# galatolofederico/clip-glass

Hardware: AMD Instinct MI355X
Metric: candidate latents scored/sec (GAN→CLIP fitness), StyleGAN2_ffhq_d pop=64 (higher is better)
Workload: dtype f16; 1 GPU; StyleGAN2_ffhq_d: StyleGAN2 config-f 1024px G+D + CLIP ViT-B/32, pop=64 per GPU, batch_size=4, n_obj=2; pop_per_gpu=64, global_pop=64, batch_size=4, parallelism=population-shard x1, device=AMD Radeon Graphics (gfx950:sramecc+:xnack-), 256 CUs, hbm_gib=288

## Files before the change

clip_glass_amd/csrc/conv_down64.hip:

```cpp
#include "common.h"
#include "kernels.h"

namespace {
constexpr int TW = 29, CIN = 64, COUT = 128;
constexpr int ROWB = 64 * 128;
constexpr int V_BYTES = 4 * ROWB;
constexpr int A_BYTES = 8 * ROWB;
constexpr int XS_BYTES = 2 * 32 * 128;
constexpr int O_BYTES = 2 * 32 * 256;
constexpr int OFF_A = V_BYTES, OFF_XS = OFF_A + A_BYTES, OFF_O = OFF_XS + XS_BYTES, OFF_C = OFF_O + O_BYTES;
constexpr int LDS_BYTES = OFF_C + COUT * 4;

__device__ __forceinline__ int vaddr(int row, int col, int cg) { return row * ROWB + ((col ^ ((col >> 2) & 1)) << 7) + (cg << 4); }
__device__ __forceinline__ int aaddr(int rslot, int slot, int lc) { return rslot * ROWB + (slot << 7) + ((lc ^ ((slot >> 1) & 7)) << 4); }
__device__ __forceinline__ int oaddr(int row, int px, int c16) { return row * (32 * 256) + (px << 8) + ((c16 ^ (px & 15)) << 4); }
__device__ __forceinline__ h8 fir4(h8 a, h8 b, h8 c, h8 d) {
    const half_t q = (half_t)0.125f, t = (half_t)0.375f;
    const h8 k125 = {q, q, q, q, q, q, q, q}, k375 = {t, t, t, t, t, t, t, t};
    return __builtin_elementwise_fma(b + c, k375, (a + d) * k125);
}
__device__ __forceinline__ int opaque(int v) { asm volatile("" : "+v"(v)); return v; }
__device__ __forceinline__ int uni(int v) { return __builtin_amdgcn_readfirstlane(v); }
struct RSet { h8 a[4]; h8 x; int b, tx, s, valid; };
}

struct Down64Params {
    const half_t* h;
    const half_t* xs;
    const half_t* w1;
    const half_t* ws;
    const float* b1;
    half_t* y;
    int B, R;
};

__global__ __launch_bounds__(512, 1) void conv_down64_kernel(Down64Params p, int tiles_x, int SY, int n_steps, int per_block) {
    extern __shared__ __attribute__((aligned(16))) char smem[];
    char* Vs = smem;
    char* As = smem + OFF_A;
    char* Xs = smem + OFF_XS;
    char* Os = smem + OFF_O;
    float* Cb = (float*)(smem + OFF_C);
    const int R = p.R, Ro = R >> 1;
    const int first = blockIdx.x * per_block;
    const int last = min(first + per_block, n_steps);
    if (first >= last) return;
    const h8 zero = {0, 0, 0, 0, 0, 0, 0, 0};

    int nx_left = last - first, nx_prime = 1, nx_b, nx_tx, nx_s;
    {
        const int per_img = tiles_x * SY;
        nx_b = uni(first / per_img);
        const int rem = first - nx_b * per_img;
        nx_tx = uni(rem / SY);
        nx_s = uni(rem - nx_tx * SY);
    }
    const int total = nx_left + 1 + (nx_s + nx_left - 1) / SY;

    auto issue = [&](RSet& Rg) {
        Rg.b = nx_b; Rg.tx = nx_tx;
        if (nx_prime) {
            Rg.s = nx_s - 1; Rg.valid = 0; nx_prime = 0;
        } else {
            Rg.s = nx_s; Rg.valid = nx_left > 0;
            if (nx_left > 1) {
                if (++nx_s == SY) { nx_s = 0; nx_prime = 1; if (++nx_tx == tiles_x) { nx_tx = 0; ++nx_b; } }
            }
            if (nx_left > 0) --nx_left;
        }
        const int t = opaque(threadIdx.x), cg = t & 7, cs = t >> 3;
        const half_t* img = p.h + (long long)Rg.b * R * R * CIN;
        const int xo = min(max(2 * TW * Rg.tx - 2 + cs, 0), R - 1) * CIN + cg * 8;
#pragma unroll
        for (int k = 0; k < 4; ++k) {
            const int iy = min(max(4 * Rg.s + 2 + k, 0), R - 1);
            Rg.a[k] = *(const h8*)(img + iy * (R * CIN) + xo);
        }
        const int v = min(t, 2 * TW * 8 - 1), row = v >= TW * 8, rem = v - row * (TW * 8);
        const int yy = min(max(2 * Rg.s + row, 0), Ro - 1), xx = min(TW * Rg.tx + (rem >> 3), Ro - 1);
        Rg.x = *(const h8*)(p.xs + (((long long)Rg.b * Ro + yy) * Ro + xx) * CIN + (rem & 7) * 8);
    };

    h8 Wm[9][4], Wk[4];
    {
        const int t = threadIdx.x, lr = t & 31, kh = (t >> 5) & 1, nb = (t >> 6) & 3;
#pragma unroll
        for (int tap = 0; tap < 9; ++tap)
#pragma unroll
            for (int kk = 0; kk < 4; ++kk) Wm[tap][kk] = *(const h8*)(p.w1 + ((tap * COUT + nb * 32 + lr) * CIN + kk * 16 + kh * 8));
#pragma unroll
        for (int kk = 0; kk < 4; ++kk) {
            const h8 wv = *(const h8*)(p.ws + ((nb * 32 + lr) * CIN + kk * 16 + kh * 8));
#pragma unroll
            for (int q = 0; q < 8; ++q) Wk[kk][q] = (half_t)((float)wv[q] * 0.70710678118654752440f);
        }
        if (t < COUT) Cb[t] = p.b1[t];
    }

    h8 c0 = zero, c1 = zero, c2 = zero;

    auto step = [&](RSet& Rg) {
        const int b = Rg.b, tx = Rg.tx, s = Rg.s, valid = Rg.valid;
        const int ox = 2 * TW * tx - 2, oy = 4 * s + 2;
        __syncthreads();
        {
            const int t = opaque(threadIdx.x), cg = t & 7, cs = t >> 3;
            const bool border = ox < 0 || ox + 64 > R || oy < 0 || oy + 4 > R;
            if (border) {
                const bool colok = (unsigned)(ox + cs) < (unsigned)R;
#pragma unroll
                for (int k = 0; k < 4; ++k) Rg.a[k] = (colok && (unsigned)(oy + k) < (unsigned)R) ? Rg.a[k] : zero;
            }
            *(h8*)(Vs + vaddr(0, cs, cg)) = fir4(c0, c1, c2, Rg.a[0]);
            *(h8*)(Vs + vaddr(1, cs, cg)) = fir4(c1, c2, Rg.a[0], Rg.a[1]);
            *(h8*)(Vs + vaddr(2, cs, cg)) = fir4(c2, Rg.a[0], Rg.a[1], Rg.a[2]);
            *(h8*)(Vs + vaddr(3, cs, cg)) = fir4(Rg.a[0], Rg.a[1], Rg.a[2], Rg.a[3]);
            c0 = Rg.a[1]; c1 = Rg.a[2]; c2 = Rg.a[3];
            if (t < 2 * TW * 8) {
                const int row = t >= TW * 8, rem = t - row * (TW * 8);
                *(h8*)(Xs + aaddr(0, row * 32 + (rem >> 3), rem & 7)) = Rg.x;
            }
        }
        issue(Rg);
        __syncthreads();
        {
            const int t = opaque(threadIdx.x), lane = t & 63, wave = uni(t >> 6);
            const int row = wave >> 1, j = (wave & 1) * 8 + (lane >> 3), cg = lane & 7;
            if (j < 15) {
                h8 v[7];
#pragma unroll
                for (int k = 0; k < 7; ++k) v[k] = *(const h8*)(Vs + vaddr(row, 4 * j + k, cg));
                const int rslot = (4 * s + 1 + row) & 7;
#pragma unroll
                for (int i = 0; i < 4; ++i) {
                    const int c = 4 * j + i;
                    const int slot = (c & 1) ? 32 + (c >> 1) : (c >> 1);
                    *(h8*)(As + aaddr(rslot, slot, cg)) = fir4(v[i], v[i + 1], v[i + 2], v[i + 3]);
                }
            }
        }
        __syncthreads();
        const int tm = opaque(threadIdx.x), lr = tm & 31, kh = (tm >> 5) & 1, wave = uni(tm >> 6), r = wave >> 2, nb = wave & 3;
        f16x acc;
#pragma unroll
        for (int q = 0; q < 16; ++q) acc[q] = 0.f;
#pragma unroll
        for (int ky = 0; ky < 3; ++ky) {
            const int rslot = (4 * s + 2 * r + ky) & 7;
#pragma unroll
            for (int kx = 0; kx < 3; ++kx)
#pragma unroll
                for (int kk = 0; kk < 4; ++kk) {
                    const h8 xf = *(const h8*)(As + aaddr(rslot, (kx == 1 ? 32 : (kx >> 1)) + lr, kk * 2 + kh));
                    acc = mfma32(Wm[ky * 3 + kx][kk], xf, acc);
                    if (kk == 3 && (kx & 1) == (ky & 1)) __builtin_amdgcn_sched_barrier(0);
                }
        }
#pragma unroll
        for (int g = 0; g < 4; ++g) {
            const f4 bb = *(const f4*)(Cb + nb * 32 + 8 * g + 4 * kh);
#pragma unroll
            for (int q = 0; q < 4; ++q) {
                const float v = acc[g * 4 + q] + bb[q];
                acc[g * 4 + q] = fmaxf(v, 0.2f * v);
            }
        }
#pragma unroll
        for (int kk = 0; kk < 4; ++kk) acc = mfma32(Wk[kk], *(const h8*)(Xs + aaddr(0, r * 32 + lr, kk * 2 + kh)), acc);
#pragma unroll
        for (int g = 0; g < 4; ++g) {
            h4 out;
#pragma unroll
            for (int q = 0; q < 4; ++q) out[q] = (half_t)acc[g * 4 + q];
            *(h4*)(Os + oaddr(r, lr, nb * 4 + g) + kh * 8) = out;
        }
        __syncthreads();
        if (valid) {
            const int t = opaque(threadIdx.x);
            const int npx = min(TW, Ro - TW * tx);
#pragma unroll
            for (int k = 0; k < 2; ++k) {
                const int v = t + 512 * k;
                const int row = v >= TW * 16, rem = v - row * (TW * 16), px = rem >> 4, ch = rem & 15;
                if (v < 2 * TW * 16 && px < npx)
                    *(h8*)(p.y + (((long long)b * Ro + 2 * s + row) * Ro + TW * tx + px) * COUT + ch * 8) = *(const h8*)(Os + oaddr(row, px, ch));
            }
        }
    };

    RSet r0, r1;
    issue(r0);
    issue(r1);
    for (int it = 0; it < total; it += 2) {
        step(r0);
        step(r1);
    }
}

bool conv_down64_supported(int R, int Cin, int Cout) {
    return Cin == CIN && Cout == COUT && R >= 16 && R % 4 == 0 && (long long)R * R * Cin < (1LL << 31) && glass_lds_fits(LDS_BYTES);
}

const char* launch_conv_down64(const half_t* h, const half_t* xs, const half_t* w1, const half_t* ws, const float* b1, half_t* y,
                               int B, int R, int Cin, int Cout, hipStream_t st) {
    if (!conv_down64_supported(R, Cin, Cout)) return nullptr;
    Down64Params p;
    p.h = h; p.xs = xs; p.w1 = w1; p.ws = ws; p.b1 = b1; p.y = y; p.B = B; p.R = R;
    const int Ro = R / 2, tiles_x = (Ro + TW - 1) / TW, SY = Ro / 2;
    const long long steps = (long long)B * tiles_x * SY;
    if (steps >= (1LL << 30)) return nullptr;
    static DevOnce once;
    once.run([&] { (void)hipFuncSetAttribute((const void*)conv_down64_kernel, hipFuncAttributeMaxDynamicSharedMemorySize, LDS_BYTES); });
    const int slots = glass_cu_count();
    const int per_block = (int)((steps + slots - 1) / slots);
    const int grid = (int)((steps + per_block - 1) / per_block);
    hipLaunchKernelGGL(conv_down64_kernel, dim3(grid), dim3(512), LDS_BYTES, st, p, tiles_x, SY, (int)steps, per_block);
    return "conv_down64_kernel";
}
```

Before: 2182 candidates/s.

## Software-pipeline down64 conv: split waves between MFMA and FIR/store phases

Restructures the fused downsample conv kernel so the two row halves of waves work in different phases. One half runs its MFMA work while the other does output stores, vertical FIR and row prefetch, which cuts the barriers per step from four to two and raises priority for one group. The skip-connection weights move from registers into LDS, and the MFMA loop now prefetches operand fragments with explicit scheduling barriers. The aim is to overlap LDS/global traffic with matrix math and reduce register pressure, at the cost of more LDS use and a more complex, fragile schedule.

```diff
diff --git a/clip_glass_amd/csrc/conv_down64.hip b/clip_glass_amd/csrc/conv_down64.hip
--- a/clip_glass_amd/csrc/conv_down64.hip
+++ b/clip_glass_amd/csrc/conv_down64.hip
@@ -9,7 +9,9 @@
 constexpr int XS_BYTES = 2 * 32 * 128;
 constexpr int O_BYTES = 2 * 32 * 256;
 constexpr int OFF_A = V_BYTES, OFF_XS = OFF_A + A_BYTES, OFF_O = OFF_XS + XS_BYTES, OFF_C = OFF_O + O_BYTES;
-constexpr int LDS_BYTES = OFF_C + COUT * 4;
+constexpr int WK_BYTES = 4 * 4 * 64 * 16;
+constexpr int OFF_WK = OFF_C + COUT * 4;
+constexpr int LDS_BYTES = OFF_WK + WK_BYTES;
 
 __device__ __forceinline__ int vaddr(int row, int col, int cg) { return row * ROWB + ((col ^ ((col >> 2) & 1)) << 7) + (cg << 4); }
 __device__ __forceinline__ int aaddr(int rslot, int slot, int lc) { return rslot * ROWB + (slot << 7) + ((lc ^ ((slot >> 1) & 7)) << 4); }
@@ -21,7 +23,7 @@
 }
 __device__ __forceinline__ int opaque(int v) { asm volatile("" : "+v"(v)); return v; }
 __device__ __forceinline__ int uni(int v) { return __builtin_amdgcn_readfirstlane(v); }
-struct RSet { h8 a[4]; h8 x; int b, tx, s, valid; };
+struct RSet { h8 a[4]; int b, tx, s, valid; };
 }
 
 struct Down64Params {
@@ -41,6 +43,7 @@
     char* Xs = smem + OFF_XS;
     char* Os = smem + OFF_O;
     float* Cb = (float*)(smem + OFF_C);
+    char* Wks = smem + OFF_WK;
     const int R = p.R, Ro = R >> 1;
     const int first = blockIdx.x * per_block;
     const int last = min(first + per_block, n_steps);
@@ -57,7 +60,7 @@
     }
     const int total = nx_left + 1 + (nx_s + nx_left - 1) / SY;
 
-    auto issue = [&](RSet& Rg) {
+    auto issue_rows = [&](RSet& Rg) {
         Rg.b = nx_b; Rg.tx = nx_tx;
         if (nx_prime) {
             Rg.s = nx_s - 1; Rg.valid = 0; nx_prime = 0;
@@ -76,12 +79,16 @@
             const int iy = min(max(4 * Rg.s + 2 + k, 0), R - 1);
             Rg.a[k] = *(const h8*)(img + iy * (R * CIN) + xo);
         }
+    };
+    h8 xv;
+    auto issue_skip = [&](const RSet& Rg) {
+        const int t = opaque(threadIdx.x);
         const int v = min(t, 2 * TW * 8 - 1), row = v >= TW * 8, rem = v - row * (TW * 8);
         const int yy = min(max(2 * Rg.s + row, 0), Ro - 1), xx = min(TW * Rg.tx + (rem >> 3), Ro - 1);
-        Rg.x = *(const h8*)(p.xs + (((long long)Rg.b * Ro + yy) * Ro + xx) * CIN + (rem & 7) * 8);
-    };
-
-    h8 Wm[9][4], Wk[4];
+        xv = *(const h8*)(p.xs + (((long long)Rg.b * Ro + yy) * Ro + xx) * CIN + (rem & 7) * 8);
+    };
+
+    h8 Wm[9][4];
     {
         const int t = threadIdx.x, lr = t & 31, kh = (t >> 5) & 1, nb = (t >> 6) & 3;
 #pragma unroll
@@ -91,70 +98,66 @@
 #pragma unroll
         for (int kk = 0; kk < 4; ++kk) {
             const h8 wv = *(const h8*)(p.ws + ((nb * 32 + lr) * CIN + kk * 16 + kh * 8));
-#pragma unroll
-            for (int q = 0; q < 8; ++q) Wk[kk][q] = (half_t)((float)wv[q] * 0.70710678118654752440f);
+            h8 wk;
+#pragma unroll
+            for (int q = 0; q < 8; ++q) wk[q] = (half_t)((float)wv[q] * 0.70710678118654752440f);
+            if (t < 256) *(h8*)(Wks + (((nb * 4 + kk) * 64 + (t & 63)) << 4)) = wk;
         }
         if (t < COUT) Cb[t] = p.b1[t];
     }
 
     h8 c0 = zero, c1 = zero, c2 = zero;
-
-    auto step = [&](RSet& Rg) {
-        const int b = Rg.b, tx = Rg.tx, s = Rg.s, valid = Rg.valid;
-        const int ox = 2 * TW * tx - 2, oy = 4 * s + 2;
-        __syncthreads();
-        {
-            const int t = opaque(threadIdx.x), cg = t & 7, cs = t >> 3;
-            const bool border = ox < 0 || ox + 64 > R || oy < 0 || oy + 4 > R;
-            if (border) {
-                const bool colok = (unsigned)(ox + cs) < (unsigned)R;
-#pragma unroll
-                for (int k = 0; k < 4; ++k) Rg.a[k] = (colok && (unsigned)(oy + k) < (unsigned)R) ? Rg.a[k] : zero;
-            }
-            *(h8*)(Vs + vaddr(0, cs, cg)) = fir4(c0, c1, c2, Rg.a[0]);
-            *(h8*)(Vs + vaddr(1, cs, cg)) = fir4(c1, c2, Rg.a[0], Rg.a[1]);
-            *(h8*)(Vs + vaddr(2, cs, cg)) = fir4(c2, Rg.a[0], Rg.a[1], Rg.a[2]);
-            *(h8*)(Vs + vaddr(3, cs, cg)) = fir4(Rg.a[0], Rg.a[1], Rg.a[2], Rg.a[3]);
-            c0 = Rg.a[1]; c1 = Rg.a[2]; c2 = Rg.a[3];
-            if (t < 2 * TW * 8) {
-                const int row = t >= TW * 8, rem = t - row * (TW * 8);
-                *(h8*)(Xs + aaddr(0, row * 32 + (rem >> 3), rem & 7)) = Rg.x;
-            }
-        }
-        issue(Rg);
-        __syncthreads();
-        {
-            const int t = opaque(threadIdx.x), lane = t & 63, wave = uni(t >> 6);
-            const int row = wave >> 1, j = (wave & 1) * 8 + (lane >> 3), cg = lane & 7;
-            if (j < 15) {
-                h8 v[7];
-#pragma unroll
-                for (int k = 0; k < 7; ++k) v[k] = *(const h8*)(Vs + vaddr(row, 4 * j + k, cg));
-                const int rslot = (4 * s + 1 + row) & 7;
-#pragma unroll
-                for (int i = 0; i < 4; ++i) {
-                    const int c = 4 * j + i;
-                    const int slot = (c & 1) ? 32 + (c >> 1) : (c >> 1);
-                    *(h8*)(As + aaddr(rslot, slot, cg)) = fir4(v[i], v[i + 1], v[i + 2], v[i + 3]);
-                }
-            }
-        }
-        __syncthreads();
-        const int tm = opaque(threadIdx.x), lr = tm & 31, kh = (tm >> 5) & 1, wave = uni(tm >> 6), r = wave >> 2, nb = wave & 3;
+    struct Meta { int b, tx, s, valid; };
+
+    auto vfir = [&](RSet& Rg, Meta& m) {
+        m.b = Rg.b; m.tx = Rg.tx; m.s = Rg.s; m.valid = Rg.valid;
+        const int ox = 2 * TW * Rg.tx - 2, oy = 4 * Rg.s + 2;
+        const int t = opaque(threadIdx.x), cg = t & 7, cs = t >> 3;
+        const bool border = ox < 0 || ox + 64 > R || oy < 0 || oy + 4 > R;
+        if (border) {
+            const bool colok = (unsigned)(ox + cs) < (unsigned)R;
+#pragma unroll
+            for (int k = 0; k < 4; ++k) Rg.a[k] = (colok && (unsigned)(oy + k) < (unsigned)R) ? Rg.a[k] : zero;
+        }
+        *(h8*)(Vs + vaddr(0, cs, cg)) = fir4(c0, c1, c2, Rg.a[0]);
+        *(h8*)(Vs + vaddr(1, cs, cg)) = fir4(c1, c2, Rg.a[0], Rg.a[1]);
+        *(h8*)(Vs + vaddr(2, cs, cg)) = fir4(c2, Rg.a[0], Rg.a[1], Rg.a[2]);
+        *(h8*)(Vs + vaddr(3, cs, cg)) = fir4(Rg.a[0], Rg.a[1], Rg.a[2], Rg.a[3]);
+        c0 = Rg.a[1]; c1 = Rg.a[2]; c2 = Rg.a[3];
+    };
+    auto store_rows = [&](const Meta& m) {
+        if (m.valid) {
+            const int t = opaque(threadIdx.x);
+            const int npx = min(TW, Ro - TW * m.tx);
+#pragma unroll
+            for (int k = 0; k < 4; ++k) {
+                const int v = t + 256 * k;
+                const int row = v >= TW * 16, rem = v - row * (TW * 16), px = rem >> 4, ch = rem & 15;
+                if (v < 2 * TW * 16 && px < npx)
+                    *(h8*)(p.y + (((long long)m.b * Ro + 2 * m.s + row) * Ro + TW * m.tx + px) * COUT + ch * 8) = *(const h8*)(Os + oaddr(row, px, ch));
+            }
+        }
+    };
+    auto mfma_run = [&](int s, int r, h4 (&out)[4]) {
         f16x acc;
+        const int tm = opaque(threadIdx.x), lr = tm & 31, kh = (tm >> 5) & 1, nb = uni(tm >> 6) & 3;
 #pragma unroll
         for (int q = 0; q < 16; ++q) acc[q] = 0.f;
-#pragma unroll
-        for (int ky = 0; ky < 3; ++ky) {
-            const int rslot = (4 * s + 2 * r + ky) & 7;
-#pragma unroll
-            for (int kx = 0; kx < 3; ++kx)
-#pragma unroll
-                for (int kk = 0; kk < 4; ++kk) {
-                    const h8 xf = *(const h8*)(As + aaddr(rslot, (kx == 1 ? 32 : (kx >> 1)) + lr, kk * 2 + kh));
-                    acc = mfma32(Wm[ky * 3 + kx][kk], xf, acc);
-                    if (kk == 3 && (kx & 1) == (ky & 1)) __builtin_amdgcn_sched_barrier(0);
-                }
+        const int a0 = (lr << 7) + ((kh ^ ((lr >> 1) & 7)) << 4), a2 = ((lr + 1) << 7) + ((kh ^ (((lr + 1) >> 1) & 7)) << 4);
+        auto frag = [&](int i) -> h8 {
+            if (i >= 36) return *(const h8*)(Xs + r * (32 * 128) + (opaque(a0) ^ ((i - 36) << 5)));
+            const int ky = i / 12, kx = (i >> 2) % 3, kk = i & 3;
+            return *(const h8*)(As + ((4 * s + 2 * r + ky) & 7) * ROWB + (kx == 1 ? 32 * 128 : 0) + (opaque(kx == 2 ? a2 : a0) ^ (kk << 5)));
+        };
+        auto wfrag = [&](int kk) -> h8 { return *(const h8*)(Wks + (((nb * 4 + kk) * 64 + (tm & 63)) << 4)); };
+        h8 f[4];
+#pragma unroll
+        for (int i = 0; i < 4; ++i) f[i] = frag(i);
+#pragma unroll
+        for (int i = 0; i < 36; ++i) {
+            acc = mfma32(Wm[i >> 2][i & 3], f[i & 3], acc);
+            f[i & 3] = i < 34 ? frag(i + 4) : wfrag(i - 34);
+            __builtin_amdgcn_sched_barrier(0);
         }
 #pragma unroll
         for (int g = 0; g < 4; ++g) {
@@ -165,36 +168,81 @@
                 acc[g * 4 + q] = fmaxf(v, 0.2f * v);
             }
         }
-#pragma unroll
-        for (int kk = 0; kk < 4; ++kk) acc = mfma32(Wk[kk], *(const h8*)(Xs + aaddr(0, r * 32 + lr, kk * 2 + kh)), acc);
-#pragma unroll
-        for (int g = 0; g < 4; ++g) {
-            h4 out;
-#pragma unroll
-            for (int q = 0; q < 4; ++q) out[q] = (half_t)acc[g * 4 + q];
-            *(h4*)(Os + oaddr(r, lr, nb * 4 + g) + kh * 8) = out;
-        }
+        __builtin_amdgcn_sched_barrier(0);
+        acc = mfma32(f[2], f[0], acc);
+        f[2] = wfrag(2); f[0] = frag(38);
+        __builtin_amdgcn_sched_barrier(0);
+        acc = mfma32(f[3], f[1], acc);
+        f[3] = wfrag(3); f[1] = frag(39);
+        __builtin_amdgcn_sched_barrier(0);
+        acc = mfma32(f[2], f[0], acc);
+        acc = mfma32(f[3], f[1], acc);
+#pragma unroll
+        for (int g = 0; g < 4; ++g)
+#pragma unroll
+            for (int q = 0; q < 4; ++q) out[g][q] = (half_t)acc[g * 4 + q];
+    };
+    auto write_out = [&](const h4 (&out)[4]) {
+        const int t = opaque(threadIdx.x), lr = t & 31, kh = (t >> 5) & 1, wave = uni(t >> 6), nb = wave & 3;
+#pragma unroll
+        for (int g = 0; g < 4; ++g) *(h4*)(Os + oaddr(wave >> 2, lr, nb * 4 + g) + kh * 8) = out[g];
+    };
+    auto phase_b = [&](const RSet& Nx, int s) {
+        const int t = opaque(threadIdx.x), lane = t & 63, wave = uni(t >> 6);
+        if (t < 2 * TW * 8) {
+            const int row = t >= TW * 8, rem = t - row * (TW * 8);
+            *(h8*)(Xs + aaddr(0, row * 32 + (rem >> 3), rem & 7)) = xv;
+        }
+        issue_skip(Nx);
+        __builtin_amdgcn_sched_barrier(0);
+        const int row = wave >> 1, j = (wave & 1) * 8 + (lane >> 3), cg = lane & 7;
+        if (j < 15) {
+            h8 v[7];
+#pragma unroll
+            for (int k = 0; k < 7; ++k) v[k] = *(const h8*)(Vs + vaddr(row, 4 * j + k, cg));
+            const int rslot = (4 * s + 1 + row) & 7;
+#pragma unroll
+            for (int i = 0; i < 4; ++i) {
+                const int c = 4 * j + i;
+                const int slot = (c & 1) ? 32 + (c >> 1) : (c >> 1);
+                *(h8*)(As + aaddr(rslot, slot, cg)) = fir4(v[i], v[i + 1], v[i + 2], v[i + 3]);
+            }
+        }
+    };
+
+    const int r = uni(threadIdx.x >> 8);
+    Meta prv = {0, 0, 0, 0}, cur, nxt;
+    h4 out[4];
+    RSet r0, r1;
+    issue_rows(r0); issue_skip(r0);
+    issue_rows(r1);
+    vfir(r0, cur);
+    issue_rows(r0);
+    __syncthreads();
+    phase_b(r1, cur.s);
+    __syncthreads();
+    if (r) __builtin_amdgcn_s_setprio(1);
+
+    auto step = [&](RSet& Rg, const RSet& Nx) {
+        if (r == 1) mfma_run(cur.s, 1, out);
+        __builtin_amdgcn_sched_barrier(0);
+        if (r == 0) store_rows(prv);
+        __builtin_amdgcn_sched_barrier(0);
+        vfir(Rg, nxt);
+        issue_rows(Rg);
+        __builtin_amdgcn_sched_barrier(0);
+        if (r == 0) mfma_run(cur.s, 0, out);
         __syncthreads();
-        if (valid) {
-            const int t = opaque(threadIdx.x);
-            const int npx = min(TW, Ro - TW * tx);
-#pragma unroll
-            for (int k = 0; k < 2; ++k) {
-                const int v = t + 512 * k;
-                const int row = v >= TW * 16, rem = v - row * (TW * 16), px = rem >> 4, ch = rem & 15;
-                if (v < 2 * TW * 16 && px < npx)
-                    *(h8*)(p.y + (((long long)b * Ro + 2 * s + row) * Ro + TW * tx + px) * COUT + ch * 8) = *(const h8*)(Os + oaddr(row, px, ch));
-            }
-        }
-    };
-
-    RSet r0, r1;
-    issue(r0);
-    issue(r1);
+        write_out(out);
+        phase_b(Nx, nxt.s);
+        __syncthreads();
+        prv = cur; cur = nxt;
+    };
     for (int it = 0; it < total; it += 2) {
-        step(r0);
-        step(r1);
+        step(r1, r0);
+        step(r0, r1);
     }
+    if (r == 0) store_rows(prv);
 }
 
 bool conv_down64_supported(int R, int Cin, int Cout) {
```

New measurement: 2193 candidates/s (median of 6 runs). About the same (+0.5%).
